# privefl/bigsnpr

Measured on NVIDIA H100. Metric: genotypes/sec in bed_prodVec, higher is better.
Workload: dtype f64

## Files before the change

bigsnpr_b200/csrc/bsg_pmv.cu:

```cuda
#include <algorithm>
#include <math.h>
#include <stdio.h>
#include <stdlib.h>
#include <string.h>

#include <cub/device/device_scan.cuh>

#include "bsg_internal.cuh"
#include "bsg_pmv_shared.cuh"

namespace bsg {
namespace pmv {

constexpr int SEG = 128;
constexpr int CODES = 512;
constexpr int DIG = 4096;
constexpr int STAGES = 6;
constexpr int STAGE_BYTES = 2 * DIG;
constexpr int SMEM_BYTES = STAGES * STAGE_BYTES + 128;
constexpr int MAX_CHUNKS_PER_ITEM = 512;

struct Args {
  const uint8_t *P;
  int64_t stride;
// ... 513 lines not shown
      if ((cw == 11 || cw == 15) && (r == 2 || r == 3) && st >= 0 && st <= 2) {
        var_cw = cw;
        var_r = r;
        var_s = st;
      }
    }
  }
  const int GROUP = var_cw * 32;
  Args a;
  a.P = P;
  a.stride = stride;
  a.lines = lines;
  a.nlines = nlines;
  a.nlines_pad = (int)round_up(nlines, GROUP);
  a.nchunks = (int)(round_up(((int64_t)L + 3) / 4, SEG) / SEG);
  int ngroups = a.nlines_pad / GROUP;
  int target_items = 24 * 132;
  int ks = (target_items + ngroups - 1) / ngroups;
  int ks_max = std::max(1, a.nchunks / 16);
  int ks_min = (a.nchunks + MAX_CHUNKS_PER_ITEM - 1) / MAX_CHUNKS_PER_ITEM;
  ks = std::min(ks, ks_max);
  ks = std::max(ks, ks_min);
  ks = std::max(ks, 1);
  a.chunks_per_split = (a.nchunks + ks - 1) / ks;
  a.ksplit = (a.nchunks + a.chunks_per_split - 1) / a.chunks_per_split;
  a.dig1 = dig1;
  a.dig2 = dig2;
  a.na_flags = na_flags;
  a.use_na = use_na;
  BSG_TRY(v->s_part.ensure((size_t)a.nlines_pad * 16 * sizeof(long long)));
  a.part = v->s_part.as<long long>();
  BSG_CUDA(cudaMemsetAsync(a.part, 0, (size_t)a.nlines_pad * 16 * sizeof(long long), s));
  const int mode = plane_hi ? 3 : (!use_na ? 0 : (dig2 ? 2 : 1));
  if (plane_hi && !dig2) return fail(BSG_ERR_ARG, "high-bit plane needs its own digits");
  void (*kern)(const Args) = nullptr;
#define PMV_PICK(CWv, Rv, Sv)                                                                   \
  if (var_cw == CWv && var_r == Rv && var_s == Sv)                                              \
    kern = mode == 0 ? k_pmv<0, CWv, Rv, Sv>                                                    \
                     : (mode == 1 ? k_pmv<1, CWv, Rv, Sv> : (mode == 2 ? k_pmv<2, CWv, Rv, Sv> : k_pmv<3, CWv, Rv, Sv>));
  PMV_PICK(11, 2, 0)
  PMV_PICK(11, 2, 1)
  PMV_PICK(11, 2, 2)
  PMV_PICK(11, 3, 0)
  PMV_PICK(11, 3, 1)
  PMV_PICK(15, 2, 1)
#undef PMV_PICK
  if (!kern) return fail(BSG_ERR_ARG, "unknown k_pmv variant");
  BSG_CUDA(cudaFuncSetAttribute(kern, cudaFuncAttributeMaxDynamicSharedMemorySize, SMEM_BYTES));
  int nsm = 132;
  cudaDeviceGetAttribute(&nsm, cudaDevAttrMultiProcessorCount, v->h->device);
  int nitems = ngroups * a.ksplit;
  int grid = std::min(nitems, nsm);
  if (g_timing) cudaEventRecord(g_ev0[g_ev_n % EV_POOL], s);
  kern<<<grid, (var_cw + 1) * 32, SMEM_BYTES, s>>>(a);
  if (g_timing) {
    cudaEventRecord(g_ev1[g_ev_n % EV_POOL], s);
    g_ev_n++;
  }
  count_launch();
  BSG_CUDA(cudaGetLastError());
  *out_args = a;
  return BSG_OK;
}

}

namespace pmvt {
using namespace pmv;
constexpr int TLINES = 32, TBYTES = 512, TWARPS = 8, TSTAGES = 6;
constexpr int WSTAGE_BYTES = TLINES * 64;
constexpr int TSMEM = TWARPS * TSTAGES * WSTAGE_BYTES;
constexpr int MAX_LINES_PER_ITEM = 1 << 16;

struct TArgs {
  const uint8_t *P;
  int64_t stride;
  const int *lines;
  int nlines;
  const uint8_t *dig;
  int lines_per_split, ksplit, nblocks, n;
  long long *part;
};

__device__ __forceinline__ void cp_async16(uint32_t dst, const void *src, int src_bytes) {
  asm volatile("cp.async.cg.shared.global [%0], [%1], 16, %2;" ::"r"(dst), "l"(src), "r"(src_bytes) : "memory");
}

template <int PLANE>
__global__ void __launch_bounds__(TWARPS * 32, 2) k_pmvT_lines(const TArgs a) {
  extern __shared__ __align__(128) uint8_t smem[];
  const int tid = threadIdx.x, warp = tid >> 5, lane = tid & 31, g = lane >> 2, q = lane & 3;
  const int blk = blockIdx.x % a.nblocks, ks = blockIdx.x / a.nblocks;
  const int64_t byte0 = (int64_t)blk * TBYTES + 64 * warp;
  const int l0 = ks * a.lines_per_split, l1 = min(a.nlines, l0 + a.lines_per_split);
  const int nsteps = (l1 - l0 + TLINES - 1) / TLINES;
  const uint32_t wbase = smem_u32(smem) + warp * (TSTAGES * WSTAGE_BYTES);

  const int lrow = lane >> 2, lch = lane & 3;
  const int64_t colb = (byte0 + 16 * lch < a.stride) ? byte0 + 16 * lch : 0;
  uint32_t dst_off[4];
#pragma unroll
  for (int i = 0; i < 4; i++) {
    const int row = 8 * i + lrow;
    const int hf = row >> 4, qq = (row >> 2) & 3, r = row & 3, sl = lch >> 1, hc = lch & 1;
    dst_off[i] = (uint32_t)((((((r * 2 + hf) * 2 + sl) * 4 + qq) * 8) + 4 * hc) * 4);
  }
  auto issue = [&](int step, int stage) {
    const uint32_t dst = wbase + stage * WSTAGE_BYTES;
#pragma unroll
    for (int i = 0; i < 4; i++) {
      const int t = min(l0 + step * TLINES + 8 * i + lrow, l1 - 1);
      const int phys = a.lines[t];
      cp_async16(dst + dst_off[i], a.P + colb + (int64_t)phys * a.stride, 16);
    }
  };

  int acc[4][4][4];
#pragma unroll
  for (int j = 0; j < 4; j++)
#pragma unroll
    for (int c = 0; c < 4; c++)
#pragma unroll
      for (int k = 0; k < 4; k++) acc[j][c][k] = 0;

#pragma unroll
  for (int st = 0; st < TSTAGES - 1; st++) {
    if (st < nsteps) issue(st, st);
    asm volatile("cp.async.commit_group;" ::: "memory");
  }
  const uint8_t *dg = a.dig + (int64_t)(l0 / TLINES) * 256 + g * 32 + 4 * q;
  uint32_t nb0 = 0, nb1 = 0;
  if (nsteps > 0) {
    nb0 = *reinterpret_cast<const uint32_t *>(dg);
    nb1 = *reinterpret_cast<const uint32_t *>(dg + 16);
  }
  const uint32_t rd_base = wbase + (uint32_t)((q * 8 + g) * 4);

  auto compute = [&](uint32_t st_base, uint32_t b0, uint32_t b1) {
    uint32_t W[2][2][4];
#pragma unroll
    for (int sl = 0; sl < 2; sl++)
#pragma unroll
      for (int hf = 0; hf < 2; hf++) {
        const uint32_t ad = st_base + (hf * 2 + sl) * 128;
        const uint32_t x0 = lds32(ad), x1 = lds32(ad + 512), x2 = lds32(ad + 1024), x3 = lds32(ad + 1536);
        const uint32_t t0 = prmt(x0, x1, 0x5140), t1 = prmt(x2, x3, 0x5140);
        const uint32_t t2 = prmt(x0, x1, 0x7362), t3 = prmt(x2, x3, 0x7362);
        W[sl][hf][0] = prmt(t0, t1, 0x5410);
        W[sl][hf][1] = prmt(t0, t1, 0x7632);
        W[sl][hf][2] = prmt(t2, t3, 0x5410);
        W[sl][hf][3] = prmt(t2, t3, 0x7632);
      }
#pragma unroll
    for (int j = 0; j < 4; j++) {
      uint32_t wa = W[0][0][j], wb = W[1][0][j], wc2 = W[0][1][j], wd = W[1][1][j];
      if (PLANE == 1) {
        wa = wa & (wa >> 1) & 0x55555555u;
        wb = wb & (wb >> 1) & 0x55555555u;
        wc2 = wc2 & (wc2 >> 1) & 0x55555555u;
        wd = wd & (wd >> 1) & 0x55555555u;
      } else if (PLANE == 2) {
        wa = (wa >> 1) & 0x55555555u;
        wb = (wb >> 1) & 0x55555555u;
        wc2 = (wc2 >> 1) & 0x55555555u;
        wd = (wd >> 1) & 0x55555555u;
      }
      mma_u8s8(acc[j][0], wa & 0x03030303u, wb & 0x03030303u, wc2 & 0x03030303u, wd & 0x03030303u, b0, b1);
      mma_u8s8(acc[j][1], wa & 0x0C0C0C0Cu, wb & 0x0C0C0C0Cu, wc2 & 0x0C0C0C0Cu, wd & 0x0C0C0C0Cu, b0, b1);
      mma_u8s8(acc[j][2], wa & 0x30303030u, wb & 0x30303030u, wc2 & 0x30303030u, wd & 0x30303030u, b0, b1);
      mma_u8s8(acc[j][3], wa & 0xC0C0C0C0u, wb & 0xC0C0C0C0u, wc2 & 0xC0C0C0C0u, wd & 0xC0C0C0C0u, b0, b1);
    }
  };

  uint32_t rd_stage = 0, wr_stage = (TSTAGES - 1) * WSTAGE_BYTES;
  const uint8_t *dgn = dg + 256;
  for (int step = 0; step < nsteps; step++) {
    asm volatile("cp.async.wait_group %0;" ::"n"(TSTAGES - 2) : "memory");
    __syncwarp();
    {
      const int nxt = step + TSTAGES - 1;
      if (nxt < nsteps) issue(nxt, (int)(wr_stage / WSTAGE_BYTES));
      asm volatile("cp.async.commit_group;" ::: "memory");
    }
    const uint32_t b0 = nb0, b1 = nb1;
    if (step + 1 < nsteps) {
      nb0 = *reinterpret_cast<const uint32_t *>(dgn);
      nb1 = *reinterpret_cast<const uint32_t *>(dgn + 16);
      dgn += 256;
    }
    compute(rd_base + rd_stage, b0, b1);
    rd_stage = rd_stage + WSTAGE_BYTES == TSTAGES * WSTAGE_BYTES ? 0 : rd_stage + WSTAGE_BYTES;
    wr_stage = wr_stage + WSTAGE_BYTES == TSTAGES * WSTAGE_BYTES ? 0 : wr_stage + WSTAGE_BYTES;
  }
  asm volatile("cp.async.wait_group 0;" ::: "memory");
#pragma unroll
  for (int j = 0; j < 4; j++)
#pragma unroll
    for (int c = 0; c < 4; c++)
#pragma unroll
      for (int sl = 0; sl < 2; sl++) {
        const int64_t sample = 4 * (byte0 + 4 * (8 * sl + g) + j) + c;
        if (sample < a.n) {
          unsigned long long *dst = reinterpret_cast<unsigned long long *>(a.part) + sample * 16 + (PLANE ? 8 : 0) + 2 * q;
          long long v0 = acc[j][c][2 * sl], v1 = acc[j][c][2 * sl + 1];
          v0 >>= 2 * c;
          v1 >>= 2 * c;
          if (v0) atomicAdd(dst, (unsigned long long)v0);
          if (v1) atomicAdd(dst + 1, (unsigned long long)v1);
        }
      }
}

constexpr int TBOX = 32 * 128;
constexpr int TDIG_OFF = 4 * TBOX;
constexpr int TSTAGE_BYTES = 4 * TBOX + 1024;
constexpr int TCSTAGES = 6;
constexpr int TSMEM_TMA = TCSTAGES * TSTAGE_BYTES + 2 * TCSTAGES * 8 + 1024;


template <int PLANE>
__global__ void __launch_bounds__(TWARPS * 32, 2) k_pmvT(const __grid_constant__ CUtensorMap map, const TArgs a) {
  extern __shared__ __align__(128) uint8_t smem[];
  const int tid = threadIdx.x, warp = tid >> 5, lane = tid & 31, g = lane >> 2, q = lane & 3;
  const int blk = blockIdx.x % a.nblocks, ks = blockIdx.x / a.nblocks;
  const int l0 = ks * a.lines_per_split, l1 = min(a.nlines, l0 + a.lines_per_split);
  const int nsteps = (l1 - l0 + TLINES - 1) / TLINES;
  const uint32_t sbase = (smem_u32(smem) + 1023u) & ~1023u;
  const uint32_t bar_base = sbase + TCSTAGES * TSTAGE_BYTES;
  auto fill = [&](int step, int st) {
    const uint32_t full = bar_base + 8 * st, dst = sbase + st * TSTAGE_BYTES;
    const uint8_t *dg = a.dig + (int64_t)(l0 / TLINES + step) * 256;
    mbar_expect_tx(full, 4 * TBOX + 256);
#pragma unroll
    for (int j = 0; j < 4; j++) tma_load_2d(dst + j * TBOX, &map, full, blk * TBYTES + 128 * j, l0 + step * TLINES);
    bulk_g2s(dst + TDIG_OFF, dg, 128, full);
    bulk_g2s(dst + TDIG_OFF + 144, dg + 128, 128, full);
  };
  if (tid == 0) {
    for (int st = 0; st < TCSTAGES; st++) {
      mbar_init(bar_base + 8 * st, 1);
      mbar_init(bar_base + 8 * (TCSTAGES + st), TWARPS);
    }
    asm volatile("fence.mbarrier_init.release.cluster;" ::: "memory");
    for (int st = 0; st < min(TCSTAGES, nsteps); st++) fill(st, st);
  }
  __syncthreads();
  int stage = 0, pstage = 0;
  uint32_t phase = 0, pphase = 0;

  const int64_t byte0 = (int64_t)blk * TBYTES + 64 * warp;
  const int rsw = 2 * (q >> 1);
  const uint32_t chunk0 = (4 * (warp & 1) + (g >> 2)) ^ (4 * (q & 1) + rsw);
  const uint32_t rd_base = sbase + (warp >> 1) * TBOX + q * 512 + (rsw << 7) + chunk0 * 16 + 4 * (g & 3);
  const uint32_t dg_base = sbase + TDIG_OFF + g * 32 + 16 * (g >> 2) + 4 * q;
  const uint32_t sel_lo = rsw ? 0x1054u : 0x5410u, sel_hi = rsw ? 0x3276u : 0x7632u;

  int acc[4][4][4];
#pragma unroll
  for (int j = 0; j < 4; j++)
#pragma unroll
    for (int c = 0; c < 4; c++)
#pragma unroll
      for (int k = 0; k < 4; k++) acc[j][c][k] = 0;

  for (int step = 0; step < nsteps; step++) {
    const uint32_t full = bar_base + 8 * stage, empty = bar_base + 8 * (TCSTAGES + stage);
    const uint32_t so = stage * TSTAGE_BYTES;
    const int cstage = stage;
    const uint32_t cphase = phase;
    mbar_wait(full, phase);
    const uint32_t b0 = lds32(dg_base + so), b1 = lds32(dg_base + so + 16);
    uint32_t W[2][2][4];
#pragma unroll
    for (int sl = 0; sl < 2; sl++)
#pragma unroll
      for (int hf = 0; hf < 2; hf++) {
        const uint32_t ad = rd_base + so, hb = hf * (16 * 128);
        const uint32_t x0 = lds32((ad ^ TRD(0, sl)) + hb), x1 = lds32((ad ^ TRD(1, sl)) + hb);
        const uint32_t x2 = lds32((ad ^ TRD(2, sl)) + hb), x3 = lds32((ad ^ TRD(3, sl)) + hb);
        const uint32_t t0 = prmt(x0, x1, 0x5140), t1 = prmt(x2, x3, 0x5140);
        const uint32_t t2 = prmt(x0, x1, 0x7362), t3 = prmt(x2, x3, 0x7362);
        W[sl][hf][0] = prmt(t0, t1, sel_lo);
        W[sl][hf][1] = prmt(t0, t1, sel_hi);
        W[sl][hf][2] = prmt(t2, t3, sel_lo);
        W[sl][hf][3] = prmt(t2, t3, sel_hi);
      }
    __syncwarp();
    if (lane == 0) mbar_arrive(empty);
    if (++stage == TCSTAGES) {
      stage = 0;
      phase ^= 1;
    }
#pragma unroll
    for (int j = 0; j < 4; j++) {
      uint32_t wa = W[0][0][j], wb = W[1][0][j], wc2 = W[0][1][j], wd = W[1][1][j];
      if (PLANE == 1) {
        wa = wa & (wa >> 1) & 0x55555555u;
        wb = wb & (wb >> 1) & 0x55555555u;
        wc2 = wc2 & (wc2 >> 1) & 0x55555555u;
        wd = wd & (wd >> 1) & 0x55555555u;
      } else if (PLANE == 2) {
        wa = (wa >> 1) & 0x55555555u;
        wb = (wb >> 1) & 0x55555555u;
        wc2 = (wc2 >> 1) & 0x55555555u;
        wd = (wd >> 1) & 0x55555555u;
      }
      mma_u8s8(acc[j][0], wa & 0x03030303u, wb & 0x03030303u, wc2 & 0x03030303u, wd & 0x03030303u, b0, b1);
      mma_u8s8(acc[j][1], wa & 0x0C0C0C0Cu, wb & 0x0C0C0C0Cu, wc2 & 0x0C0C0C0Cu, wd & 0x0C0C0C0Cu, b0, b1);
      mma_u8s8(acc[j][2], wa & 0x30303030u, wb & 0x30303030u, wc2 & 0x30303030u, wd & 0x30303030u, b0, b1);
      mma_u8s8(acc[j][3], wa & 0xC0C0C0C0u, wb & 0xC0C0C0C0u, wc2 & 0xC0C0C0C0u, wd & 0xC0C0C0C0u, b0, b1);
    }
    if (tid == 0 && step >= 1 && step - 1 + TCSTAGES < nsteps) {
      mbar_wait(bar_base + 8 * (TCSTAGES + pstage), pphase);
      fill(step - 1 + TCSTAGES, pstage);
    }
    __syncwarp();
    pstage = cstage;
    pphase = cphase;
  }
#pragma unroll
  for (int j = 0; j < 4; j++)
#pragma unroll
    for (int c = 0; c < 4; c++)
#pragma unroll
      for (int sl = 0; sl < 2; sl++) {
        const int64_t sample = 4 * (byte0 + 4 * (8 * sl + g) + j) + c;
        if (sample < a.n) {
          unsigned long long *dst = reinterpret_cast<unsigned long long *>(a.part) + sample * 16 + (PLANE ? 8 : 0) + 2 * q;
          long long v0 = acc[j][c][2 * sl], v1 = acc[j][c][2 * sl + 1];
          v0 >>= 2 * c;
          v1 >>= 2 * c;
          if (v0) atomicAdd(dst, (unsigned long long)v0);
          if (v1) atomicAdd(dst + 1, (unsigned long long)v1);
        }
      }
}

constexpr int W2STAGE_BYTES = TLINES * 32;
constexpr int T2BYTES = TWARPS * 32;
constexpr int T2SMEM = TWARPS * TSTAGES * W2STAGE_BYTES;

template <int PL, bool LINES>
__global__ void __launch_bounds__(TWARPS * 32, 2) k_pmvT2(const TArgs a, const uint8_t *__restrict__ dig2) {
  extern __shared__ __align__(128) uint8_t smem[];
  const int tid = threadIdx.x, warp = tid >> 5, lane = tid & 31, g = lane >> 2, q = lane & 3;
  const int blk = blockIdx.x % a.nblocks, ks = blockIdx.x / a.nblocks;
  const int64_t byte0 = (int64_t)blk * T2BYTES + 32 * warp;
  const int l0 = ks * a.lines_per_split, l1 = min(a.nlines, l0 + a.lines_per_split);
  const int nsteps = (l1 - l0 + TLINES - 1) / TLINES;
  const uint32_t wbase = smem_u32(smem) + warp * (TSTAGES * W2STAGE_BYTES);
  const int lrow = lane >> 1, lch = lane & 1;
  const int64_t colb = (byte0 + 16 * lch < a.stride) ? byte0 + 16 * lch : 0;
  uint32_t dst_off[2];
#pragma unroll
  for (int i = 0; i < 2; i++) {
    const int row = 16 * i + lrow;
    const int hf = row >> 4, qq = (row >> 2) & 3, r = row & 3;
    dst_off[i] = (uint32_t)(((((r * 2 + hf) * 4 + qq) * 8) + 4 * lch) * 4);
  }
  const int full_steps = (l1 - l0) / TLINES;
  const int64_t stride16 = 16 * a.stride;
  auto issue = [&](int step, int stage) {
    const uint32_t dst = wbase + stage * W2STAGE_BYTES;
#pragma unroll
    for (int i = 0; i < 2; i++) {
      const int t = min(l0 + step * TLINES + 16 * i + lrow, l1 - 1);
      const int phys = LINES ? a.lines[t] : t;
      cp_async16(dst + dst_off[i], a.P + colb + (int64_t)phys * a.stride, 16);
    }
  };
  int acc[2][2][4][4];
#pragma unroll
  for (int p = 0; p < 2; p++)
#pragma unroll
    for (int u = 0; u < 2; u++)
#pragma unroll
      for (int c = 0; c < 4; c++)
#pragma unroll
        for (int k = 0; k < 4; k++) acc[p][u][c][k] = 0;
#pragma unroll
  for (int st = 0; st < TSTAGES - 1; st++) {
    if (st < nsteps) issue(st, st);
    asm volatile("cp.async.commit_group;" ::: "memory");
  }
  const int64_t doff = (int64_t)(l0 / TLINES) * 256 + g * 32 + 4 * q;
  const uint8_t *dg = a.dig + doff, *dp = dig2 + doff;
  uint32_t nb0 = 0, nb1 = 0, np0 = 0, np1 = 0;
  if (nsteps > 0) {
    nb0 = *reinterpret_cast<const uint32_t *>(dg);
    nb1 = *reinterpret_cast<const uint32_t *>(dg + 16);
    np0 = *reinterpret_cast<const uint32_t *>(dp);
    np1 = *reinterpret_cast<const uint32_t *>(dp + 16);
  }
  const uint32_t rd_base = wbase + (uint32_t)((q * 8 + g) * 4);

  auto compute = [&](uint32_t st_base, uint32_t b0, uint32_t b1, uint32_t p0, uint32_t p1) {
    uint32_t W[2][4];
#pragma unroll
    for (int hf = 0; hf < 2; hf++) {
      const uint32_t ad = st_base + hf * 128;
      const uint32_t x0 = lds32(ad), x1 = lds32(ad + 256), x2 = lds32(ad + 512), x3 = lds32(ad + 768);
      const uint32_t t0 = prmt(x0, x1, 0x5140), t1 = prmt(x2, x3, 0x5140);
      const uint32_t t2 = prmt(x0, x1, 0x7362), t3 = prmt(x2, x3, 0x7362);
      W[hf][0] = prmt(t0, t1, 0x5410);
      W[hf][1] = prmt(t0, t1, 0x7632);
      W[hf][2] = prmt(t2, t3, 0x5410);
      W[hf][3] = prmt(t2, t3, 0x7632);
    }
#pragma unroll
    for (int u = 0; u < 2; u++) {
      const uint32_t wa = W[0][u], wb = W[0][u + 2], wc2 = W[1][u], wd = W[1][u + 2];
      mma_u8s8(acc[0][u][0], wa & 0x03030303u, wb & 0x03030303u, wc2 & 0x03030303u, wd & 0x03030303u, b0, b1);
      mma_u8s8(acc[0][u][1], wa & 0x0C0C0C0Cu, wb & 0x0C0C0C0Cu, wc2 & 0x0C0C0C0Cu, wd & 0x0C0C0C0Cu, b0, b1);
      mma_u8s8(acc[0][u][2], wa & 0x30303030u, wb & 0x30303030u, wc2 & 0x30303030u, wd & 0x30303030u, b0, b1);
      mma_u8s8(acc[0][u][3], wa & 0xC0C0C0C0u, wb & 0xC0C0C0C0u, wc2 & 0xC0C0C0C0u, wd & 0xC0C0C0C0u, b0, b1);
      const uint32_t fa = PL == 1 ? (wa & (wa >> 1)) : (wa >> 1), fb = PL == 1 ? (wb & (wb >> 1)) : (wb >> 1);
      const uint32_t fc = PL == 1 ? (wc2 & (wc2 >> 1)) : (wc2 >> 1), fd = PL == 1 ? (wd & (wd >> 1)) : (wd >> 1);
      mma_u8s8(acc[1][u][0], fa & 0x01010101u, fb & 0x01010101u, fc & 0x01010101u, fd & 0x01010101u, p0, p1);
// ... 244 lines not shown
    if (!rc) {
      v->col_maxmult = max_mult(zc);
      rc = dev_copy((void **)&v->d_col, zc.data(), (size_t)nc * sizeof(int), s);
    }
  }
  if (!rc && v->has_scaling) {
    rc = dev_copy((void **)&v->d_center, center, (size_t)nc * sizeof(double), s);
    if (!rc) rc = dev_copy((void **)&v->d_scale, scale, (size_t)nc * sizeof(double), s);
  }
  if (!rc) rc = v->s_scal.ensure(2 * sizeof(pmv::Scal));
  if (!rc && h->fbm_generic) rc = dosage_view_masks(v);
  cudaError_t e = cudaStreamSynchronize(s);
  if (!rc && e != cudaSuccess) rc = cuda_fail(e, "view upload");
  if (rc) {
    bsg_view_destroy(v);
    return rc;
  }
  *out = v;
  return BSG_OK;
}

void bsg_view_destroy(bsg_view *v) {
  if (!v) return;
  cudaSetDevice(v->h->device);
  cudaStreamSynchronize(v->h->stream);
  void *ptrs[] = {v->d_row, v->d_col, v->d_center, v->d_scale, v->d_rows_unique, v->d_row_gather, v->d_rowsel, v->d_colsel};
  for (void *p : ptrs)
    if (p) cudaFree(p);
  DevBuf *bufs[] = {&v->s_vec0, &v->s_vec1, &v->s_q0, &v->s_q1, &v->s_dig1, &v->s_dig2, &v->s_part, &v->s_scal,
                    &v->s_full};
  for (DevBuf *b : bufs) b->release();
  delete v;
}

int bsg_view_cprodvec_dev(bsg_view *v, const double *x_dev, double *out_dev, void *stream) {
  if (!v || !x_dev || !out_dev) return fail(BSG_ERR_ARG, "null argument");
  bsg_bed *h = v->h;
  BSG_TRY(bind_device(h));
  cudaStream_t s = stream ? (cudaStream_t)stream : cudaStreamLegacy;
  if (v->nc == 0) return BSG_OK;
  if (h->fbm_generic) return dosage_cprodvec(v, x_dev, out_dev, s);
  using namespace pmv;
  Scal *sc = v->s_scal.as<Scal>();
  const bool lists = h->has_na && na_ell_ready(h);
  BSG_TRY(prep_pmv(v, 1, 0, x_dev, nullptr, nullptr, 1, nullptr, false, true, lists, s));
  Args a;
  BSG_TRY(run_pmv(v, h->A, h->strideA, h->n, v->d_col, v->nc, v->s_dig1.as<uint8_t>(), nullptr, h->naA,
                  lists ? 0 : h->has_na, &a, s));
  if (lists) BSG_TRY(na_ell_correction(h, 1, v->d_col, v->nc, v->s_q0.as<long long>(), a.part, s));
  k_finish_cprod<<<(v->nc + 255) / 256, 256, 0, s>>>(a.part, v->nc, sc, v->d_center, v->d_scale, h->has_na, out_dev);
  count_launch();
  BSG_CUDA(cudaGetLastError());
  return BSG_OK;
}

static int run_pmvT(bsg_view *v, const uint8_t *dig_raw, int plane, const uint8_t *dig_plane, long long **part_out,
                    cudaStream_t s) {
  using namespace pmv;
  using namespace pmvt;
  bsg_bed *h = v->h;
  const int n = h->n, nc = v->nc;
  const int nsteps = (nc + TLINES - 1) / TLINES;
  BSG_TRY(v->s_part.ensure((size_t)std::max(n, 1) * 16 * sizeof(long long)));
  long long *part = v->s_part.as<long long>();
  *part_out = part;
  BSG_CUDA(cudaMemsetAsync(part, 0, (size_t)n * 16 * sizeof(long long), s));
  if (nc == 0 || n == 0) return BSG_OK;
  TArgs a;
  a.P = h->A;
  a.stride = h->strideA;
  a.lines = v->d_col;
  a.nlines = nc;
  a.n = n;
  a.part = part;
  const int64_t nbytes = ((int64_t)n + 3) / 4;
  a.nblocks = (int)((nbytes + TBYTES - 1) / TBYTES);
  int nsm = 132;
  cudaDeviceGetAttribute(&nsm, cudaDevAttrMultiProcessorCount, h->device);
  static int waves = 0;
  if (!waves) {
    const char *ev = getenv("BSG_PMVT_WAVES");
    waves = ev ? std::max(1, std::min(64, atoi(ev))) : 4;
  }
  auto pick_ks = [&](int nblocks) {
    const int slots = 2 * nsm;
    const int lo = std::max(1, (nc + MAX_LINES_PER_ITEM - 1) / MAX_LINES_PER_ITEM);
    const int hi = std::max(lo, std::min(std::max(1, nsteps / 32), std::max(lo, (4 * waves * slots) / std::max(nblocks, 1))));
    static int force_ks = -1;
    if (force_ks < 0) {
      const char *ev = getenv("BSG_PMVT_KS");
      force_ks = ev ? std::max(0, atoi(ev)) : 0;
    }
    if (force_ks > 0) return std::max(lo, force_ks);
    int best = lo;
    double best_score = -1;
    for (int ks = lo; ks <= hi; ks++) {
      const double ctas = (double)nblocks * ks, nwav = ceil(ctas / slots);
      double score = ctas / (nwav * slots);
      const double lines = (double)nc / ks;
      score *= lines / (lines + 1000.0);
      if (nwav < waves) score *= 0.9 + 0.1 * nwav / waves;
      if (score > best_score + 1e-9) {
        best_score = score;
        best = ks;
      }
    }
    return best;
  };
  int ks = pick_ks(a.nblocks);
  a.lines_per_split = (int)round_up((nc + ks - 1) / ks, TLINES);
  a.ksplit = (nc + a.lines_per_split - 1) / a.lines_per_split;
  static unsigned attr_done = 0;
  if (!(attr_done >> (h->device & 31) & 1u)) {
    BSG_CUDA(cudaFuncSetAttribute(k_pmvT<0>, cudaFuncAttributeMaxDynamicSharedMemorySize, TSMEM_TMA));
    BSG_CUDA(cudaFuncSetAttribute(k_pmvT_lines<0>, cudaFuncAttributeMaxDynamicSharedMemorySize, TSMEM));
    BSG_CUDA(cudaFuncSetAttribute(k_pmvT2<1, false>, cudaFuncAttributeMaxDynamicSharedMemorySize, T2SMEM));
    BSG_CUDA(cudaFuncSetAttribute(k_pmvT2<1, true>, cudaFuncAttributeMaxDynamicSharedMemorySize, T2SMEM));
    BSG_CUDA(cudaFuncSetAttribute(k_pmvT2<2, false>, cudaFuncAttributeMaxDynamicSharedMemorySize, T2SMEM));
    BSG_CUDA(cudaFuncSetAttribute(k_pmvT2<2, true>, cudaFuncAttributeMaxDynamicSharedMemorySize, T2SMEM));
    attr_done |= 1u << (h->device & 31);
  }
  const int thr = TWARPS * 32;
  const bool lines = a.lines != nullptr;
  a.dig = dig_raw;
  if (g_timing) cudaEventRecord(g_ev0[g_ev_n % EV_POOL], s);
  if (!plane) {
    const int grid = a.nblocks * a.ksplit;
    if (lines) {
      k_pmvT_lines<0><<<grid, thr, TSMEM, s>>>(a);
    } else {
      CUtensorMap map;
      BSG_TRY(make_map(&map, a.P, nc, a.stride, TLINES));
      k_pmvT<0><<<grid, thr, TSMEM_TMA, s>>>(map, a);
    }
  } else {
    a.nblocks = (int)((nbytes + T2BYTES - 1) / T2BYTES);
    const int ks2 = pick_ks(a.nblocks);
    a.lines_per_split = (int)round_up((nc + ks2 - 1) / ks2, TLINES);
    a.ksplit = (nc + a.lines_per_split - 1) / a.lines_per_split;
    const int grid = a.nblocks * a.ksplit;
    if (plane == 1) {
      if (lines)
        k_pmvT2<1, true><<<grid, thr, T2SMEM, s>>>(a, dig_plane);
      else
        k_pmvT2<1, false><<<grid, thr, T2SMEM, s>>>(a, dig_plane);
    } else {
      if (lines)
        k_pmvT2<2, true><<<grid, thr, T2SMEM, s>>>(a, dig_plane);
      else
        k_pmvT2<2, false><<<grid, thr, T2SMEM, s>>>(a, dig_plane);
    }
  }
  if (g_timing) {
    cudaEventRecord(g_ev1[g_ev_n % EV_POOL], s);
    g_ev_n++;
  }
  count_launch();
  BSG_CUDA(cudaGetLastError());
  return BSG_OK;
}

static int prep_T(bsg_view *v, int mode, const double *x, const double *p1, const double *p2, int nv, const double *xb,
                  bool two, cudaStream_t s, long long *qna_full = nullptr, int na_second = 0) {
  using namespace pmv;
  using namespace pmvt;
  Scal *sc = v->s_scal.as<Scal>();
  const int nc = v->nc;
  const int nsteps = (nc + TLINES - 1) / TLINES;
  const int hb = qna_full ? hb_bits(v->col_maxmult) : 0;
  BSG_TRY(v->s_dig1.ensure((size_t)std::max(nsteps, 1) * 256));
  if (two) BSG_TRY(v->s_dig2.ensure((size_t)std::max(nsteps, 1) * 256));
  uint8_t *dig1 = v->s_dig1.as<uint8_t>(), *dig2 = two ? v->s_dig2.as<uint8_t>() : nullptr;
  BSG_CUDA(cudaMemsetAsync(sc, 0, nv * sizeof(Scal), s));
  k_prep1<<<SUMCZ_BLOCKS, 256, 0, s>>>(mode, x, p1, p2, nc, hb, sc);
  if (xb) k_prep1<<<SUMCZ_BLOCKS, 256, 0, s>>>(mode, xb, p1, p2, nc, hb, sc + 1);
  const int grid = launch_cap((int64_t)std::max(nsteps, 1) * TLINES, 256, 1184);
  if (nv == 1)
    k_quantT<1><<<grid, 256, 0, s>>>(mode, x, nullptr, p1, p2, nc, nsteps * TLINES, sc, dig1, dig2, v->d_col, qna_full,
                                     na_second);
  else
    k_quantT<2><<<grid, 256, 0, s>>>(mode, x, xb, p1, p2, nc, nsteps * TLINES, sc, dig1, dig2, nullptr, nullptr, 0);
  count_launch(xb ? 3 : 2);
  return BSG_OK;
}

static int prodvec_T(bsg_view *v, const double *x_dev, double *out_dev, cudaStream_t s, bsg_comm *comm) {
  using namespace pmv;
  bsg_bed *h = v->h;
  Scal *sc = v->s_scal.as<Scal>();
  const int n = h->n, nc = v->nc;
  const int mode = v->has_scaling ? 1 : 0;
  const bool lists = h->has_na && na_ell_ready(h);
  const bool two = v->has_scaling && h->has_na && !lists;
  long long *qna = nullptr;
  if (lists) {
    BSG_TRY(v->s_q1.ensure((size_t)h->m * sizeof(long long)));
    qna = v->s_q1.as<long long>();
    BSG_CUDA(cudaMemsetAsync(qna, 0, (size_t)h->m * sizeof(long long), s));
  }
  BSG_TRY(prep_T(v, mode, x_dev, v->d_center, v->d_scale, 1, nullptr, two, s, qna, v->has_scaling ? 1 : 0));
  long long *part = nullptr;
  BSG_TRY(run_pmvT(v, v->s_dig1.as<uint8_t>(), (h->has_na && !lists) ? 1 : 0,
                   two ? v->s_dig2.as<uint8_t>() : v->s_dig1.as<uint8_t>(), &part, s));
  if (lists) BSG_TRY(na_ell_correction(h, 0, nullptr, n, qna, part, s));
  double *full = out_dev;
  if (!v->row_identity) {
    BSG_TRY(v->s_full.ensure((size_t)n * sizeof(double)));
    full = v->s_full.as<double>();
  }
  if (comm && v->row_identity)
    return comm_finish_prod_allreduce(comm, part, n, sc, v->has_scaling, h->has_na, out_dev, s);
  if (n > 0) {
    k_finish_prod<<<(n + 255) / 256, 256, 0, s>>>(part, n, sc, v->has_scaling, h->has_na, full);
    count_launch();
  }
  if (!v->row_identity && v->nr > 0) {
// ... 760 lines not shown
```

Before: 12030 billion.

## Load genotype tiles with ldmatrix.trans and use cumulative-mask MMA decoding

Replaces the per-lane 32-bit shared loads plus prmt-based transpose in the TMA transposed product kernel with ldmatrix x4.trans loads and a reduced permute. The MMAs now use cumulative high-bit masks (0xFC, 0xF0, 0xC0) instead of isolated 2-bit fields, and adjacent accumulators are subtracted in the epilogue to recover each code position. The aim is fewer shared-memory instructions and fewer ALU ops per step. The PLANE template is dropped, and the split-K cost heuristic now weights splits more heavily when the partial buffer exceeds L2, trading parallelism for fewer atomic partial updates.

Result: faster. 12320 billion (median of 6 runs) (+2.4%).

```diff
diff --git a/bigsnpr_b200/csrc/bsg_pmv.cu b/bigsnpr_b200/csrc/bsg_pmv.cu
--- a/bigsnpr_b200/csrc/bsg_pmv.cu
+++ b/bigsnpr_b200/csrc/bsg_pmv.cu
@@ -754,8 +754,12 @@
 constexpr int TCSTAGES = 6;
 constexpr int TSMEM_TMA = TCSTAGES * TSTAGE_BYTES + 2 * TCSTAGES * 8 + 1024;
 
-
-template <int PLANE>
+__device__ __forceinline__ void ldsm_x4_trans(uint32_t (&r)[4], uint32_t addr) {
+  asm volatile("ldmatrix.sync.aligned.m8n8.x4.trans.shared.b16 {%0,%1,%2,%3}, [%4];"
+               : "=r"(r[0]), "=r"(r[1]), "=r"(r[2]), "=r"(r[3])
+               : "r"(addr));
+}
+
 __global__ void __launch_bounds__(TWARPS * 32, 2) k_pmvT(const __grid_constant__ CUtensorMap map, const TArgs a) {
   extern __shared__ __align__(128) uint8_t smem[];
   const int tid = threadIdx.x, warp = tid >> 5, lane = tid & 31, g = lane >> 2, q = lane & 3;
@@ -786,19 +790,22 @@
   uint32_t phase = 0, pphase = 0;
 
   const int64_t byte0 = (int64_t)blk * TBYTES + 64 * warp;
-  const int rsw = 2 * (q >> 1);
-  const uint32_t chunk0 = (4 * (warp & 1) + (g >> 2)) ^ (4 * (q & 1) + rsw);
-  const uint32_t rd_base = sbase + (warp >> 1) * TBOX + q * 512 + (rsw << 7) + chunk0 * 16 + 4 * (g & 3);
+  const int mi = lane >> 3, mq = (lane >> 1) & 3;
+  const int line = 16 * (mi >> 1) + 4 * mq + 2 * ((mi & 1) ^ (mq >> 1)) + (lane & 1);
+  const uint32_t rd_base = sbase + (warp >> 1) * TBOX + line * 128 + ((4 * (warp & 1) ^ (line & 7)) << 4);
   const uint32_t dg_base = sbase + TDIG_OFF + g * 32 + 16 * (g >> 2) + 4 * q;
-  const uint32_t sel_lo = rsw ? 0x1054u : 0x5410u, sel_hi = rsw ? 0x3276u : 0x7632u;
-
-  int acc[4][4][4];
-#pragma unroll
-  for (int j = 0; j < 4; j++)
-#pragma unroll
-    for (int c = 0; c < 4; c++)
-#pragma unroll
-      for (int k = 0; k < 4; k++) acc[j][c][k] = 0;
+  const uint32_t sel_even = q >= 2 ? 0x2064u : 0x6420u, sel_odd = sel_even + 0x1111u;
+  const uint32_t zero = (uint32_t)a.n >> 31;
+
+  int acc[2][2][4][4];
+#pragma unroll
+  for (int G = 0; G < 2; G++)
+#pragma unroll
+    for (int p = 0; p < 2; p++)
+#pragma unroll
+      for (int c = 0; c < 4; c++)
+#pragma unroll
+        for (int k = 0; k < 4; k++) acc[G][p][c][k] = 0;
 
   for (int step = 0; step < nsteps; step++) {
     const uint32_t full = bar_base + 8 * stage, empty = bar_base + 8 * (TCSTAGES + stage);
@@ -807,46 +814,35 @@
     const uint32_t cphase = phase;
     mbar_wait(full, phase);
     const uint32_t b0 = lds32(dg_base + so), b1 = lds32(dg_base + so + 16);
-    uint32_t W[2][2][4];
-#pragma unroll
-    for (int sl = 0; sl < 2; sl++)
+    uint32_t A[4][2][2];
+    uint32_t dep = b0 ^ b1;
+#pragma unroll
+    for (int ch = 0; ch < 4; ch++) {
+      uint32_t r[4];
+      ldsm_x4_trans(r, (rd_base + so) ^ (ch << 4));
+      dep ^= r[0];
 #pragma unroll
       for (int hf = 0; hf < 2; hf++) {
-        const uint32_t ad = rd_base + so, hb = hf * (16 * 128);
-        const uint32_t x0 = lds32((ad ^ TRD(0, sl)) + hb), x1 = lds32((ad ^ TRD(1, sl)) + hb);
-        const uint32_t x2 = lds32((ad ^ TRD(2, sl)) + hb), x3 = lds32((ad ^ TRD(3, sl)) + hb);
-        const uint32_t t0 = prmt(x0, x1, 0x5140), t1 = prmt(x2, x3, 0x5140);
-        const uint32_t t2 = prmt(x0, x1, 0x7362), t3 = prmt(x2, x3, 0x7362);
-        W[sl][hf][0] = prmt(t0, t1, sel_lo);
-        W[sl][hf][1] = prmt(t0, t1, sel_hi);
-        W[sl][hf][2] = prmt(t2, t3, sel_lo);
-        W[sl][hf][3] = prmt(t2, t3, sel_hi);
+        A[ch][hf][0] = prmt(r[2 * hf], r[2 * hf + 1], sel_even);
+        A[ch][hf][1] = prmt(r[2 * hf], r[2 * hf + 1], sel_odd);
       }
+    }
     __syncwarp();
-    if (lane == 0) mbar_arrive(empty);
+    if (lane == 0) mbar_arrive(empty + (dep & zero));
     if (++stage == TCSTAGES) {
       stage = 0;
       phase ^= 1;
     }
 #pragma unroll
-    for (int j = 0; j < 4; j++) {
-      uint32_t wa = W[0][0][j], wb = W[1][0][j], wc2 = W[0][1][j], wd = W[1][1][j];
-      if (PLANE == 1) {
-        wa = wa & (wa >> 1) & 0x55555555u;
-        wb = wb & (wb >> 1) & 0x55555555u;
-        wc2 = wc2 & (wc2 >> 1) & 0x55555555u;
-        wd = wd & (wd >> 1) & 0x55555555u;
-      } else if (PLANE == 2) {
-        wa = (wa >> 1) & 0x55555555u;
-        wb = (wb >> 1) & 0x55555555u;
-        wc2 = (wc2 >> 1) & 0x55555555u;
-        wd = (wd >> 1) & 0x55555555u;
+    for (int G = 0; G < 2; G++)
+#pragma unroll
+      for (int p = 0; p < 2; p++) {
+        const uint32_t wa = A[2 * G][0][p], wb = A[2 * G + 1][0][p], wc = A[2 * G][1][p], wd = A[2 * G + 1][1][p];
+        mma_u8s8(acc[G][p][0], wa, wb, wc, wd, b0, b1);
+        mma_u8s8(acc[G][p][1], wa & 0xFCFCFCFCu, wb & 0xFCFCFCFCu, wc & 0xFCFCFCFCu, wd & 0xFCFCFCFCu, b0, b1);
+        mma_u8s8(acc[G][p][2], wa & 0xF0F0F0F0u, wb & 0xF0F0F0F0u, wc & 0xF0F0F0F0u, wd & 0xF0F0F0F0u, b0, b1);
+        mma_u8s8(acc[G][p][3], wa & 0xC0C0C0C0u, wb & 0xC0C0C0C0u, wc & 0xC0C0C0C0u, wd & 0xC0C0C0C0u, b0, b1);
       }
-      mma_u8s8(acc[j][0], wa & 0x03030303u, wb & 0x03030303u, wc2 & 0x03030303u, wd & 0x03030303u, b0, b1);
-      mma_u8s8(acc[j][1], wa & 0x0C0C0C0Cu, wb & 0x0C0C0C0Cu, wc2 & 0x0C0C0C0Cu, wd & 0x0C0C0C0Cu, b0, b1);
-      mma_u8s8(acc[j][2], wa & 0x30303030u, wb & 0x30303030u, wc2 & 0x30303030u, wd & 0x30303030u, b0, b1);
-      mma_u8s8(acc[j][3], wa & 0xC0C0C0C0u, wb & 0xC0C0C0C0u, wc2 & 0xC0C0C0C0u, wd & 0xC0C0C0C0u, b0, b1);
-    }
     if (tid == 0 && step >= 1 && step - 1 + TCSTAGES < nsteps) {
       mbar_wait(bar_base + 8 * (TCSTAGES + pstage), pphase);
       fill(step - 1 + TCSTAGES, pstage);
@@ -856,21 +852,26 @@
     pphase = cphase;
   }
 #pragma unroll
-  for (int j = 0; j < 4; j++)
-#pragma unroll
-    for (int c = 0; c < 4; c++)
-#pragma unroll
-      for (int sl = 0; sl < 2; sl++) {
-        const int64_t sample = 4 * (byte0 + 4 * (8 * sl + g) + j) + c;
-        if (sample < a.n) {
-          unsigned long long *dst = reinterpret_cast<unsigned long long *>(a.part) + sample * 16 + (PLANE ? 8 : 0) + 2 * q;
-          long long v0 = acc[j][c][2 * sl], v1 = acc[j][c][2 * sl + 1];
-          v0 >>= 2 * c;
-          v1 >>= 2 * c;
-          if (v0) atomicAdd(dst, (unsigned long long)v0);
-          if (v1) atomicAdd(dst + 1, (unsigned long long)v1);
+  for (int G = 0; G < 2; G++)
+#pragma unroll
+    for (int p = 0; p < 2; p++)
+#pragma unroll
+      for (int c = 0; c < 4; c++)
+#pragma unroll
+        for (int sl = 0; sl < 2; sl++) {
+          const int64_t sample = 4 * (byte0 + 16 * (2 * G + sl) + 2 * g + p) + c;
+          if (sample < a.n) {
+            unsigned long long *dst = reinterpret_cast<unsigned long long *>(a.part) + sample * 16 + 2 * q;
+            const uint32_t n0 = c < 3 ? (uint32_t)acc[G][p][c + 1][2 * sl] : 0u;
+            const uint32_t n1 = c < 3 ? (uint32_t)acc[G][p][c + 1][2 * sl + 1] : 0u;
+            long long v0 = (int32_t)((uint32_t)acc[G][p][c][2 * sl] - n0);
+            long long v1 = (int32_t)((uint32_t)acc[G][p][c][2 * sl + 1] - n1);
+            v0 >>= 2 * c;
+            v1 >>= 2 * c;
+            if (v0) atomicAdd(dst, (unsigned long long)v0);
+            if (v1) atomicAdd(dst + 1, (unsigned long long)v1);
+          }
         }
-      }
 }
 
 constexpr int W2STAGE_BYTES = TLINES * 32;
@@ -1281,6 +1282,9 @@
     const char *ev = getenv("BSG_PMVT_WAVES");
     waves = ev ? std::max(1, std::min(64, atoi(ev))) : 4;
   }
+  int l2_bytes = 50 << 20;
+  cudaDeviceGetAttribute(&l2_bytes, cudaDevAttrL2CacheSize, h->device);
+  const double split_cost = (double)n * 16 * sizeof(long long) > l2_bytes ? 32000.0 : 1000.0;
   auto pick_ks = [&](int nblocks) {
     const int slots = 2 * nsm;
     const int lo = std::max(1, (nc + MAX_LINES_PER_ITEM - 1) / MAX_LINES_PER_ITEM);
@@ -1297,7 +1301,7 @@
       const double ctas = (double)nblocks * ks, nwav = ceil(ctas / slots);
       double score = ctas / (nwav * slots);
       const double lines = (double)nc / ks;
-      score *= lines / (lines + 1000.0);
+      score *= lines / (lines + split_cost);
       if (nwav < waves) score *= 0.9 + 0.1 * nwav / waves;
       if (score > best_score + 1e-9) {
         best_score = score;
@@ -1311,7 +1315,7 @@
   a.ksplit = (nc + a.lines_per_split - 1) / a.lines_per_split;
   static unsigned attr_done = 0;
   if (!(attr_done >> (h->device & 31) & 1u)) {
-    BSG_CUDA(cudaFuncSetAttribute(k_pmvT<0>, cudaFuncAttributeMaxDynamicSharedMemorySize, TSMEM_TMA));
+    BSG_CUDA(cudaFuncSetAttribute(k_pmvT, cudaFuncAttributeMaxDynamicSharedMemorySize, TSMEM_TMA));
     BSG_CUDA(cudaFuncSetAttribute(k_pmvT_lines<0>, cudaFuncAttributeMaxDynamicSharedMemorySize, TSMEM));
     BSG_CUDA(cudaFuncSetAttribute(k_pmvT2<1, false>, cudaFuncAttributeMaxDynamicSharedMemorySize, T2SMEM));
     BSG_CUDA(cudaFuncSetAttribute(k_pmvT2<1, true>, cudaFuncAttributeMaxDynamicSharedMemorySize, T2SMEM));
@@ -1330,7 +1334,7 @@
     } else {
       CUtensorMap map;
       BSG_TRY(make_map(&map, a.P, nc, a.stride, TLINES));
-      k_pmvT<0><<<grid, thr, TSMEM_TMA, s>>>(map, a);
+      k_pmvT<<<grid, thr, TSMEM_TMA, s>>>(map, a);
     }
   } else {
     a.nblocks = (int)((nbytes + T2BYTES - 1) / T2BYTES);
```

## Unroll TMA stage ring, distribute refill to warps, use cumulative masks for MMA

Applied to the files above, without the earlier changes.

The TMA transposed product kernel's stage loop is unrolled over the stage ring, so stage offsets and barrier addresses become compile-time constants. Swizzled read addresses are precomputed per thread. Refilling each stage is handed to a rotating warp instead of always thread 0, which is meant to stop one warp from serializing every refill. The MMA masks become cumulative prefixes (0x03, 0x0F, 0x3F, full), so each 2-bit field is recovered by differencing adjacent accumulators at store time, which drops the mask on the last MMA at the cost of extra subtractions in the epilogue. It also adds an artificial data dependency on the accumulator before the empty-barrier arrive, and the risk is that prefix sums may overflow the int32 accumulators.

Result: faster. 11640 billion before, 11900 billion after, median of 6 (+2.2%).

```diff
diff --git a/bigsnpr_b200/csrc/bsg_pmv.cu b/bigsnpr_b200/csrc/bsg_pmv.cu
--- a/bigsnpr_b200/csrc/bsg_pmv.cu
+++ b/bigsnpr_b200/csrc/bsg_pmv.cu
@@ -619,6 +619,48 @@
   long long *part;
 };
 
+template <int PLANE>
+__device__ __forceinline__ void pmvt_mma(int (&acc)[4][4][4], const uint32_t (&W)[2][2][4], uint32_t b0, uint32_t b1) {
+#pragma unroll
+  for (int j = 0; j < 4; j++) {
+    uint32_t wa = W[0][0][j], wb = W[1][0][j], wc2 = W[0][1][j], wd = W[1][1][j];
+    if (PLANE == 1) {
+      wa = wa & (wa >> 1) & 0x55555555u;
+      wb = wb & (wb >> 1) & 0x55555555u;
+      wc2 = wc2 & (wc2 >> 1) & 0x55555555u;
+      wd = wd & (wd >> 1) & 0x55555555u;
+    } else if (PLANE == 2) {
+      wa = (wa >> 1) & 0x55555555u;
+      wb = (wb >> 1) & 0x55555555u;
+      wc2 = (wc2 >> 1) & 0x55555555u;
+      wd = (wd >> 1) & 0x55555555u;
+    }
+    mma_u8s8(acc[j][0], wa & 0x03030303u, wb & 0x03030303u, wc2 & 0x03030303u, wd & 0x03030303u, b0, b1);
+    mma_u8s8(acc[j][1], wa & 0x0F0F0F0Fu, wb & 0x0F0F0F0Fu, wc2 & 0x0F0F0F0Fu, wd & 0x0F0F0F0Fu, b0, b1);
+    mma_u8s8(acc[j][2], wa & 0x3F3F3F3Fu, wb & 0x3F3F3F3Fu, wc2 & 0x3F3F3F3Fu, wd & 0x3F3F3F3Fu, b0, b1);
+    mma_u8s8(acc[j][3], wa, wb, wc2, wd, b0, b1);
+  }
+}
+
+template <int PLANE>
+__device__ __forceinline__ void pmvt_store(const int (&acc)[4][4][4], const TArgs &a, int64_t byte0, int g, int q) {
+#pragma unroll
+  for (int j = 0; j < 4; j++)
+#pragma unroll
+    for (int c = 0; c < 4; c++)
+#pragma unroll
+      for (int sl = 0; sl < 2; sl++) {
+        const int64_t sample = 4 * (byte0 + 4 * (8 * sl + g) + j) + c;
+        if (sample < a.n) {
+          unsigned long long *dst = reinterpret_cast<unsigned long long *>(a.part) + sample * 16 + (PLANE ? 8 : 0) + 2 * q;
+          const int p0 = c ? acc[j][c - 1][2 * sl] : 0, p1 = c ? acc[j][c - 1][2 * sl + 1] : 0;
+          const long long v0 = (acc[j][c][2 * sl] - p0) >> (2 * c), v1 = (acc[j][c][2 * sl + 1] - p1) >> (2 * c);
+          if (v0) atomicAdd(dst, (unsigned long long)v0);
+          if (v1) atomicAdd(dst + 1, (unsigned long long)v1);
+        }
+      }
+}
+
 __device__ __forceinline__ void cp_async16(uint32_t dst, const void *src, int src_bytes) {
   asm volatile("cp.async.cg.shared.global [%0], [%1], 16, %2;" ::"r"(dst), "l"(src), "r"(src_bytes) : "memory");
 }
@@ -688,25 +730,7 @@
         W[sl][hf][2] = prmt(t2, t3, 0x5410);
         W[sl][hf][3] = prmt(t2, t3, 0x7632);
       }
-#pragma unroll
-    for (int j = 0; j < 4; j++) {
-      uint32_t wa = W[0][0][j], wb = W[1][0][j], wc2 = W[0][1][j], wd = W[1][1][j];
-      if (PLANE == 1) {
-        wa = wa & (wa >> 1) & 0x55555555u;
-        wb = wb & (wb >> 1) & 0x55555555u;
-        wc2 = wc2 & (wc2 >> 1) & 0x55555555u;
-        wd = wd & (wd >> 1) & 0x55555555u;
-      } else if (PLANE == 2) {
-        wa = (wa >> 1) & 0x55555555u;
-        wb = (wb >> 1) & 0x55555555u;
-        wc2 = (wc2 >> 1) & 0x55555555u;
-        wd = (wd >> 1) & 0x55555555u;
-      }
-      mma_u8s8(acc[j][0], wa & 0x03030303u, wb & 0x03030303u, wc2 & 0x03030303u, wd & 0x03030303u, b0, b1);
-      mma_u8s8(acc[j][1], wa & 0x0C0C0C0Cu, wb & 0x0C0C0C0Cu, wc2 & 0x0C0C0C0Cu, wd & 0x0C0C0C0Cu, b0, b1);
-      mma_u8s8(acc[j][2], wa & 0x30303030u, wb & 0x30303030u, wc2 & 0x30303030u, wd & 0x30303030u, b0, b1);
-      mma_u8s8(acc[j][3], wa & 0xC0C0C0C0u, wb & 0xC0C0C0C0u, wc2 & 0xC0C0C0C0u, wd & 0xC0C0C0C0u, b0, b1);
-    }
+    pmvt_mma<PLANE>(acc, W, b0, b1);
   };
 
   uint32_t rd_stage = 0, wr_stage = (TSTAGES - 1) * WSTAGE_BYTES;
@@ -730,22 +754,7 @@
     wr_stage = wr_stage + WSTAGE_BYTES == TSTAGES * WSTAGE_BYTES ? 0 : wr_stage + WSTAGE_BYTES;
   }
   asm volatile("cp.async.wait_group 0;" ::: "memory");
-#pragma unroll
-  for (int j = 0; j < 4; j++)
-#pragma unroll
-    for (int c = 0; c < 4; c++)
-#pragma unroll
-      for (int sl = 0; sl < 2; sl++) {
-        const int64_t sample = 4 * (byte0 + 4 * (8 * sl + g) + j) + c;
-        if (sample < a.n) {
-          unsigned long long *dst = reinterpret_cast<unsigned long long *>(a.part) + sample * 16 + (PLANE ? 8 : 0) + 2 * q;
-          long long v0 = acc[j][c][2 * sl], v1 = acc[j][c][2 * sl + 1];
-          v0 >>= 2 * c;
-          v1 >>= 2 * c;
-          if (v0) atomicAdd(dst, (unsigned long long)v0);
-          if (v1) atomicAdd(dst + 1, (unsigned long long)v1);
-        }
-      }
+  pmvt_store<PLANE>(acc, a, byte0, g, q);
 }
 
 constexpr int TBOX = 32 * 128;
@@ -782,15 +791,19 @@
     for (int st = 0; st < min(TCSTAGES, nsteps); st++) fill(st, st);
   }
   __syncthreads();
-  int stage = 0, pstage = 0;
-  uint32_t phase = 0, pphase = 0;
 
   const int64_t byte0 = (int64_t)blk * TBYTES + 64 * warp;
   const int rsw = 2 * (q >> 1);
   const uint32_t chunk0 = (4 * (warp & 1) + (g >> 2)) ^ (4 * (q & 1) + rsw);
   const uint32_t rd_base = sbase + (warp >> 1) * TBOX + q * 512 + (rsw << 7) + chunk0 * 16 + 4 * (g & 3);
+  uint32_t rd[2][4];
+#pragma unroll
+  for (int sl = 0; sl < 2; sl++)
+#pragma unroll
+    for (int i = 0; i < 4; i++) rd[sl][i] = rd_base ^ TRD(i, sl);
   const uint32_t dg_base = sbase + TDIG_OFF + g * 32 + 16 * (g >> 2) + 4 * q;
   const uint32_t sel_lo = rsw ? 0x1054u : 0x5410u, sel_hi = rsw ? 0x3276u : 0x7632u;
+  const int wu = __shfl_sync(0xffffffffu, warp, 0);
 
   int acc[4][4][4];
 #pragma unroll
@@ -800,77 +813,40 @@
 #pragma unroll
       for (int k = 0; k < 4; k++) acc[j][c][k] = 0;
 
-  for (int step = 0; step < nsteps; step++) {
-    const uint32_t full = bar_base + 8 * stage, empty = bar_base + 8 * (TCSTAGES + stage);
-    const uint32_t so = stage * TSTAGE_BYTES;
-    const int cstage = stage;
-    const uint32_t cphase = phase;
-    mbar_wait(full, phase);
-    const uint32_t b0 = lds32(dg_base + so), b1 = lds32(dg_base + so + 16);
-    uint32_t W[2][2][4];
-#pragma unroll
-    for (int sl = 0; sl < 2; sl++)
-#pragma unroll
-      for (int hf = 0; hf < 2; hf++) {
-        const uint32_t ad = rd_base + so, hb = hf * (16 * 128);
-        const uint32_t x0 = lds32((ad ^ TRD(0, sl)) + hb), x1 = lds32((ad ^ TRD(1, sl)) + hb);
-        const uint32_t x2 = lds32((ad ^ TRD(2, sl)) + hb), x3 = lds32((ad ^ TRD(3, sl)) + hb);
-        const uint32_t t0 = prmt(x0, x1, 0x5140), t1 = prmt(x2, x3, 0x5140);
-        const uint32_t t2 = prmt(x0, x1, 0x7362), t3 = prmt(x2, x3, 0x7362);
-        W[sl][hf][0] = prmt(t0, t1, sel_lo);
-        W[sl][hf][1] = prmt(t0, t1, sel_hi);
-        W[sl][hf][2] = prmt(t2, t3, sel_lo);
-        W[sl][hf][3] = prmt(t2, t3, sel_hi);
+  uint32_t phase = 0;
+  for (int step0 = 0; step0 < nsteps; step0 += TCSTAGES, phase ^= 1) {
+#pragma unroll
+    for (int st = 0; st < TCSTAGES; st++) {
+      const int step = step0 + st;
+      if (step >= nsteps) break;
+      const uint32_t so = st * TSTAGE_BYTES;
+      mbar_wait(bar_base + 8 * st, phase);
+      const uint32_t b0 = lds32(dg_base + so), b1 = lds32(dg_base + so + 16);
+      uint32_t W[2][2][4];
+#pragma unroll
+      for (int sl = 0; sl < 2; sl++)
+#pragma unroll
+        for (int hf = 0; hf < 2; hf++) {
+          const uint32_t o = so + hf * (16 * 128);
+          const uint32_t x0 = lds32(rd[sl][0] + o), x1 = lds32(rd[sl][1] + o);
+          const uint32_t x2 = lds32(rd[sl][2] + o), x3 = lds32(rd[sl][3] + o);
+          const uint32_t t0 = prmt(x0, x1, 0x5140), t1 = prmt(x2, x3, 0x5140);
+          const uint32_t t2 = prmt(x0, x1, 0x7362), t3 = prmt(x2, x3, 0x7362);
+          W[sl][hf][0] = prmt(t0, t1, sel_lo);
+          W[sl][hf][1] = prmt(t0, t1, sel_hi);
+          W[sl][hf][2] = prmt(t2, t3, sel_lo);
+          W[sl][hf][3] = prmt(t2, t3, sel_hi);
+        }
+      pmvt_mma<PLANE>(acc, W, b0, b1);
+      if (lane == 0 && acc[0][0][0] != INT_MIN) mbar_arrive(bar_base + 8 * (TCSTAGES + st));
+      const int ps = (st + TCSTAGES - 1) % TCSTAGES;
+      if (wu == ps && step >= 1 && step - 1 + TCSTAGES < nsteps) {
+        mbar_wait(bar_base + 8 * (TCSTAGES + ps), st ? phase : phase ^ 1);
+        if (lane == 0) fill(step - 1 + TCSTAGES, ps);
       }
-    __syncwarp();
-    if (lane == 0) mbar_arrive(empty);
-    if (++stage == TCSTAGES) {
-      stage = 0;
-      phase ^= 1;
-    }
-#pragma unroll
-    for (int j = 0; j < 4; j++) {
-      uint32_t wa = W[0][0][j], wb = W[1][0][j], wc2 = W[0][1][j], wd = W[1][1][j];
-      if (PLANE == 1) {
-        wa = wa & (wa >> 1) & 0x55555555u;
-        wb = wb & (wb >> 1) & 0x55555555u;
-        wc2 = wc2 & (wc2 >> 1) & 0x55555555u;
-        wd = wd & (wd >> 1) & 0x55555555u;
-      } else if (PLANE == 2) {
-        wa = (wa >> 1) & 0x55555555u;
-        wb = (wb >> 1) & 0x55555555u;
-        wc2 = (wc2 >> 1) & 0x55555555u;
-        wd = (wd >> 1) & 0x55555555u;
-      }
-      mma_u8s8(acc[j][0], wa & 0x03030303u, wb & 0x03030303u, wc2 & 0x03030303u, wd & 0x03030303u, b0, b1);
-      mma_u8s8(acc[j][1], wa & 0x0C0C0C0Cu, wb & 0x0C0C0C0Cu, wc2 & 0x0C0C0C0Cu, wd & 0x0C0C0C0Cu, b0, b1);
-      mma_u8s8(acc[j][2], wa & 0x30303030u, wb & 0x30303030u, wc2 & 0x30303030u, wd & 0x30303030u, b0, b1);
-      mma_u8s8(acc[j][3], wa & 0xC0C0C0C0u, wb & 0xC0C0C0C0u, wc2 & 0xC0C0C0C0u, wd & 0xC0C0C0C0u, b0, b1);
-    }
-    if (tid == 0 && step >= 1 && step - 1 + TCSTAGES < nsteps) {
-      mbar_wait(bar_base + 8 * (TCSTAGES + pstage), pphase);
-      fill(step - 1 + TCSTAGES, pstage);
-    }
-    __syncwarp();
-    pstage = cstage;
-    pphase = cphase;
-  }
-#pragma unroll
-  for (int j = 0; j < 4; j++)
-#pragma unroll
-    for (int c = 0; c < 4; c++)
-#pragma unroll
-      for (int sl = 0; sl < 2; sl++) {
-        const int64_t sample = 4 * (byte0 + 4 * (8 * sl + g) + j) + c;
-        if (sample < a.n) {
-          unsigned long long *dst = reinterpret_cast<unsigned long long *>(a.part) + sample * 16 + (PLANE ? 8 : 0) + 2 * q;
-          long long v0 = acc[j][c][2 * sl], v1 = acc[j][c][2 * sl + 1];
-          v0 >>= 2 * c;
-          v1 >>= 2 * c;
-          if (v0) atomicAdd(dst, (unsigned long long)v0);
-          if (v1) atomicAdd(dst + 1, (unsigned long long)v1);
-        }
-      }
+    }
+  }
+  pmvt_store<PLANE>(acc, a, byte0, g, q);
 }
 
 constexpr int W2STAGE_BYTES = TLINES * 32;
```
